# mfkiwl/erlangnetwork-gnsslib-sdr

Hardware: AMD Instinct MI355X
Metric: correlations/sec (1 ms coh) + x real-time, 32-SV L1CA @16.368 Msps (higher is better)
Workload: dtype int8 samples x int8 carrier LUT -> int32 accumulators (exact); NCOs: the reference's fp64 running sums, bit for bit; 1 GPU; BASELINE configs[2]: 32-SV GPS L1CA tracking, 5-tap E/P/L correlators (CORRN=2, CORRD=3), 1 ms coherent, 16.368 Msps int8 IQ, per GPU; channels_per_gpu=32, epochs_per_launch=1000, taps=5, loop=open (frequencies held per launch); see closed_loop (--full), if_broadcast=none (1 GPU)

## Files before the change

erlangnetwork-gnsslib-sdr_amd/csrc/gnsscorr_api.hip:

```cpp
#include <cstdarg>
#include <cstdio>
#include <cstdlib>
#include <cstring>

#include "gnsscorr_ctx.h"

static thread_local char g_err[512] = "";

int gc_fail(int code, const char *fmt, ...)
{
    va_list ap;
    va_start(ap, fmt);
    vsnprintf(g_err, sizeof(g_err), fmt, ap);
    va_end(ap);
    return code;
}

int gc_fail_hip(hipError_t e, const char *what, const char *file, int line)
{
    snprintf(g_err, sizeof(g_err), "HIP error %d (%s) in %s at %s:%d", (int)e, hipGetErrorString(e), what,
             file, line);
    return GNSSCORR_EHIP;
}

extern "C" const char *gnsscorr_last_error(void) { return g_err; }

extern "C" int gnsscorr_device_count(void)
{
    int n = 0;
    if (hipGetDeviceCount(&n) != hipSuccess) return 0;
    return n;
}

static void destroy_handles(gnsscorr_ctx *ctx)
{
    for (auto &kv : ctx->timers)
        for (auto &p : kv.second.pending) { hipEventDestroy(p.first); hipEventDestroy(p.second); }
    for (int i = 0; i < 2; i++)
        for (hipEvent_t e : {ctx->ev_plan[i], ctx->ev_used[i], ctx->ev_corr[i], ctx->ev_fin[i]})
            if (e) hipEventDestroy(e);
    for (hipEvent_t e : {ctx->ev_spec, ctx->ev_chain, ctx->ev_pin[0], ctx->ev_pin[1], ctx->ev_in, ctx->ev_lock})
        if (e) hipEventDestroy(e);
    for (hipEvent_t e : ctx->ev_burst)
        if (e) hipEventDestroy(e);
    for (hipStream_t s : {ctx->stream_plan, ctx->stream_finish, ctx->stream_discover, ctx->stream_in})
        if (s) hipStreamDestroy(s);
    if (ctx->own_stream) hipStreamDestroy(ctx->stream);
}

extern "C" int gnsscorr_create(gnsscorr_ctx **out, int device, void *stream)
{
    if (!out) return gc_fail(GNSSCORR_EINVAL, "gnsscorr_create: null out pointer");
    int ndev = 0;
    GC_HIP(hipGetDeviceCount(&ndev));
    if (device < 0 || device >= ndev)
        return gc_fail(GNSSCORR_EHIP, "gnsscorr_create: device %d not present (%d visible)", device, ndev);
    GC_HIP(hipSetDevice(device));
    gnsscorr_ctx *ctx = new gnsscorr_ctx();
    ctx->device = device;
    hipError_t e = hipSuccess;
    if (stream) {
        ctx->stream = (hipStream_t)stream;
    } else {
        e = hipStreamCreateWithFlags(&ctx->stream, hipStreamNonBlocking);
        ctx->own_stream = e == hipSuccess;
    }
    for (hipStream_t *s : {&ctx->stream_plan, &ctx->stream_finish, &ctx->stream_discover})
        if (e == hipSuccess) e = hipStreamCreateWithFlags(s, hipStreamNonBlocking);
    for (hipEvent_t *ev : {&ctx->ev_spec, &ctx->ev_chain, &ctx->ev_plan[0], &ctx->ev_used[0], &ctx->ev_corr[0], &ctx->ev_fin[0],
                           &ctx->ev_plan[1], &ctx->ev_used[1], &ctx->ev_corr[1], &ctx->ev_fin[1]})
        if (e == hipSuccess) e = hipEventCreateWithFlags(ev, hipEventDisableTiming);
    for (hipEvent_t &ev : ctx->ev_burst)
        if (e == hipSuccess) e = hipEventCreateWithFlags(&ev, hipEventDisableTiming);
    if (e != hipSuccess) {
        destroy_handles(ctx);
        delete ctx;
        return gc_fail_hip(e, "gnsscorr_create: stream / event", __FILE__, __LINE__);
    }
    *out = ctx;
    return GNSSCORR_OK;
}

static void drop_channel_buffers(gnsscorr_ctx *ctx)
{
    gc_acq_free(ctx);
    gc_spec_free(ctx);
    ctx->dchan.reset(); ctx->dcodes.reset(); ctx->dfreqs.reset();
    ctx->state = GcTrkStateBuf();
    ctx->batch = GcBatch();
    ctx->out = GcTrkOut();
    ctx->loop = GcLoop();
    ctx->rx = GcRx();
    ctx->lock_pending = false;
}

extern "C" void gnsscorr_destroy(gnsscorr_ctx *ctx)
{
    if (!ctx) return;
    hipSetDevice(ctx->device);
    gc_quiesce(ctx, true);
    gc_acq_free(ctx);
    gc_spec_free(ctx);
    destroy_handles(ctx);
// ... 497 lines not shown
```

erlangnetwork-gnsslib-sdr_amd/csrc/gnsscorr_compat.hip:

```cpp
#include <cmath>
#include <cstdio>
#include <cstdlib>
#include <cstring>
#include <ctime>
#include <unistd.h>

#include "../../include/sdr_compat.h"
#include "gnsscorr_ctx.h"

#define SDRPRINTF printf

struct GcOnce {
    GcDevBuf<int8_t> data;
    GcDevBuf<int8_t> code;
    GcDevBuf<GcChan> chan;
    GcDevBuf<GcTrkPlan> plan;
    GcDevBuf<GcTrkUnit> unit;
    GcDevBuf<GcUnitSegs> segs;
    GcDevBuf<int> overflow;
    GcDevBuf<double> out;
    GcDevBuf<int> partial;
    GcDevBuf<GcRound> rounds;
    GcDevBuf<unsigned long long> finish;
};
// ... 33 lines not shown
        }
        *remc = gc_code_rem(c, smax, ci);
    }
}

static int corr_unit(gnsscorr_ctx *ctx, const int8_t *ring, uint64_t ringlen, int dtype, double ti,
                     int n, double freq, double phi0, double crate, double coff, const int *s, int ns,
                     const short *codein, int coden, uint64_t buffloc, double *cI, double *cQ)
{
    if (ns < 1 || 1 + 2 * ns > GNSSCORR_MAXTAPS) return gc_fail(GNSSCORR_EINVAL, "correlator: ns %d", ns);
    if (coden < 1 || coden > 1023) return gc_fail(GNSSCORR_EINVAL, "correlator: code length %d", coden);
    if (n < 1) return gc_fail(GNSSCORR_EINVAL, "correlator: n %d", n);
    int rc = once_init(ctx);
    if (rc) return rc;
    GcChan c;
    memset(&c, 0, sizeof(c));
    c.ring = ring; c.ringlen = ringlen; c.code = g_once.code;
    c.dtype = dtype; c.clen = coden; c.nsamp = n; c.ntap = 1 + 2 * ns; c.smax = s[ns - 1];
    c.tapoff[0] = 0;
    for (int k = 0; k < ns; k++) { c.tapoff[1 + 2 * k] = -s[k]; c.tapoff[2 + 2 * k] = s[k]; }
    c.ti = ti;
    GcTrkPlan p;
    memset(&p, 0, sizeof(p));
    p.buffloc = buffloc; p.coff = coff; p.phi0 = phi0; p.carrfreq = freq; p.codefreq = crate; p.n = n;
    static int8_t block[GC_CODEBLOCK];
    gc_build_codeblock(codein, coden, block, &c.nedge, &c.pm1);
    GC_HIP(hipMemcpyAsync(g_once.code, block, GC_CODEBLOCK, hipMemcpyHostToDevice, ctx->stream));
    GC_HIP(hipMemcpyAsync(g_once.chan, &c, sizeof(c), hipMemcpyHostToDevice, ctx->stream));
    GC_HIP(hipMemcpyAsync(g_once.plan, &p, sizeof(p), hipMemcpyHostToDevice, ctx->stream));
    const int nseg = gc_trk_nseg(dtype, n);
    GC_RESERVE(ctx, g_once.partial, (size_t)nseg * 2 * c.ntap);
    GC_RESERVE(ctx, g_once.rounds, (size_t)nseg * GC_MAXR);
    rc = gc_launch_trk_expand(ctx->stream, g_once.chan, g_once.plan, g_once.unit, g_once.segs, nullptr, 1, 1, g_once.rounds,
                              nseg, n, g_once.overflow);
    if (rc) return rc;
    rc = gc_launch_trk_corr(ctx->stream, g_once.chan, g_once.unit, g_once.segs, g_once.rounds, g_once.partial, 1, 1, nseg,
                            c.ntap, dtype, c.ntap, n, c.smax, nullptr);
    if (rc) return rc;
    rc = gc_launch_trk_finish(ctx->stream, g_once.partial, g_once.out, g_once.out + GNSSCORR_MAXTAPS,
                              g_once.out + 2 * GNSSCORR_MAXTAPS, g_once.out + 3 * GNSSCORR_MAXTAPS, g_once.finish, 1, 1, nseg,
                              c.ntap);
    if (rc) return rc;
    double host[2 * GNSSCORR_MAXTAPS];
    int over = 0;
    GC_HIP(hipMemcpyAsync(host, g_once.out, sizeof(host), hipMemcpyDeviceToHost, ctx->stream));
    GC_HIP(hipMemcpyAsync(&over, g_once.overflow, sizeof(int), hipMemcpyDeviceToHost, ctx->stream));
    GC_HIP(hipStreamSynchronize(ctx->stream));
    if (over) {
        GC_HIP(hipMemsetAsync(g_once.overflow, 0, sizeof(int), ctx->stream));
        return gc_fail(GNSSCORR_EINVAL, "correlator: the call spans more code periods (chip step %g x %d samples over %d chips) "
                       "or carrier binades than the NCO tables hold", ti * crate, n, coden);
    }
    memcpy(cI, host, sizeof(double) * c.ntap);
    memcpy(cQ, host + GNSSCORR_MAXTAPS, sizeof(double) * c.ntap);
    return 0;
}

extern "C" {

void correlator(const char *data, int dtype, double ti, int n, double freq, double phi0, double crate,
                double coff, int *s, int ns, double *II, double *QQ, double *remc, double *remp,
                short *codein, int coden)
{
    gnsscorr_ctx *ctx = gnsscorr_default_ctx();
    if (!ctx) { SDRPRINTF("error: correlator: no GPU context (%s)\n", gnsscorr_last_error()); return; }
    std::lock_guard<std::mutex> lk(ctx->mtx);
    if (hipSetDevice(ctx->device) != hipSuccess) { SDRPRINTF("error: correlator: hipSetDevice\n"); return; }
// ... 128 lines not shown
        const int sm = r->sdr->trk.corrp[r->sdr->trk.corrn - 1];
        if (sm > smax_max) smax_max = sm;
    }
    const int nseg = gc_trk_nseg(dtype, max_n);
    int rc = cmb_reserve(ctx, k, nseg);
    if (rc) return rc;
    const double tp0 = g_cprof.on ? CmbProf::now() : 0.0;
    const size_t plan_off = (sizeof(GcChan) * (size_t)k + 63) & ~(size_t)63;
    GcChan *hchan = reinterpret_cast<GcChan *>(q.hstage.p), *dchan = reinterpret_cast<GcChan *>(q.dstage.p);
    GcTrkPlan *hplan = reinterpret_cast<GcTrkPlan *>(q.hstage.p + plan_off), *dplan = reinterpret_cast<GcTrkPlan *>(q.dstage.p + plan_off);
    for (int i = 0; i < k; i++) {
        sdrch_t *sdr = grp[i]->sdr;
        const GcRing &ring = ctx->ring[sdr->ftype == FTYPE2 ? 1 : 0];
        CodeSlot *cs;
        rc = cmb_code(ctx, sdr, grp[i]->codesum, &cs);
        if (rc) return rc;
        GcChan &c = hchan[i];
        memset(&c, 0, sizeof(c));
        c.ring = ring.mem; c.ringlen = ring.ringlen; c.code = cs->dcode;
        c.dtype = dtype; c.clen = sdr->clen; c.nsamp = grp[i]->n; c.ntap = ntap;
        c.smax = sdr->trk.corrp[sdr->trk.corrn - 1];
        c.tapoff[0] = 0;
        for (int t = 0; t < sdr->trk.corrn; t++) { c.tapoff[1 + 2 * t] = -sdr->trk.corrp[t]; c.tapoff[2 + 2 * t] = sdr->trk.corrp[t]; }
        c.ti = sdr->ti;
        c.nedge = cs->nedge; c.pm1 = cs->pm1;
        GcTrkPlan &p = hplan[i];
        memset(&p, 0, sizeof(p));
        p.buffloc = grp[i]->buffloc; p.coff = sdr->trk.oldremcode; p.phi0 = sdr->trk.oldremcarr;
        p.carrfreq = sdr->trk.carrfreq; p.codefreq = sdr->trk.codefreq; p.n = grp[i]->n;
    }
    hipStream_t st = ctx->stream;
    const double tp1 = g_cprof.on ? CmbProf::now() : 0.0;
    GC_HIP(hipMemcpyAsync(q.dstage, q.hstage, plan_off + sizeof(GcTrkPlan) * k, hipMemcpyHostToDevice, st));
    rc = gc_launch_trk_expand(st, dchan, dplan, q.dunit, q.dsegs, nullptr, k, 1, q.drounds, nseg, max_n, q.hover.dev);
    if (rc) return rc;
    rc = gc_launch_trk_corr(st, dchan, q.dunit, q.dsegs, q.drounds, q.dpartial, k, 1, nseg, ntap, dtype, ntap, max_n, smax_max, nullptr);
    if (rc) return rc;
    double *cI = q.hres.dev, *cQ = q.hres.dev + (size_t)q.cap * ntap, *sI = q.dsum, *sQ = q.dsum + (size_t)q.cap * ntap;
    rc = gc_launch_trk_finish(st, q.dpartial, cI, cQ, sI, sQ, q.dfinish, k, 1, nseg, ntap);
    if (rc) return rc;
    const double tp2 = g_cprof.on ? CmbProf::now() : 0.0;
    GC_HIP(hipStreamSynchronize(st));
    const double tp3 = g_cprof.on ? CmbProf::now() : 0.0;
    if (*q.hover) {
        *q.hover = 0;
        return gc_fail(GNSSCORR_EINVAL, "sdrtracking: a period needs more NCO pieces than the tables hold");
    }
    for (int i = 0; i < k; i++) {
        memcpy(grp[i]->cI, q.hres + (size_t)i * ntap, sizeof(double) * ntap);
        memcpy(grp[i]->cQ, q.hres + (size_t)(q.cap + i) * ntap, sizeof(double) * ntap);
    }
    g_cmb_stats[0]++; g_cmb_stats[1] += (unsigned long long)k;
    if ((unsigned long long)k > g_cmb_stats[2]) g_cmb_stats[2] = (unsigned long long)k;
    if (g_cprof.on) {
        const double tp4 = CmbProf::now();
        g_cprof.batches++; g_cprof.reqs += (unsigned long long)k;
        g_cprof.t[0] += tp1 - tp0; g_cprof.t[1] += tp2 - tp1; g_cprof.t[2] += tp3 - tp2; g_cprof.t[3] += tp4 - tp3;
    }
    return 0;
}

void cmb_run(std::vector<TrkReq *> &batch)
{
    const double tr0 = g_cprof.on ? CmbProf::now() : 0.0;
    struct Whole { double t0; ~Whole() { if (g_cprof.on) g_cprof.t[4] += CmbProf::now() - t0; } } whole{tr0};
    gnsscorr_ctx *ctx = gnsscorr_default_ctx();
    auto fail_all = [&](std::vector<TrkReq *> &v, const char *msg) {
// ... 123 lines not shown
```

erlangnetwork-gnsslib-sdr_amd/csrc/gnsscorr_ctx.h:

```cpp
#pragma once

#include <map>
#include <mutex>
#include <string>
#include <utility>
#include <vector>

#include <cstring>
#include "gnsscorr_internal.h"

struct gnsscorr_ctx;
int gc_dev_alloc(gnsscorr_ctx *ctx, void **p, size_t bytes);

template <class T>
struct GcDevBuf {
    T *p = nullptr;
    size_t n = 0;
    GcDevBuf() = default;
    GcDevBuf(GcDevBuf &&o) noexcept : p(o.p), n(o.n) { o.p = nullptr; o.n = 0; }
    GcDevBuf &operator=(GcDevBuf &&o) noexcept
    {
        if (this != &o) { reset(); p = o.p; n = o.n; o.p = nullptr; o.n = 0; }
        return *this;
    }
// ... 65 lines not shown
    double total_ms = 0.0;
    int launches = 0;
};

struct GcAcqWork;
struct GcSpecWork;

struct GcTrkStateBuf {
    GcDevBuf<GcTrkState> buf[2];
    int icur = 0;
    bool touched = true;
    GcTrkState *cur() const { return buf[icur]; }
    GcTrkState *next() const { return buf[icur ^ 1]; }
    void commit() { icur ^= 1; }
};

struct GcTrkOut {
    GcDevBuf<double> dcorrI, dcorrQ;
    GcDevBuf<double> dsumI, dsumQ;
    GcDevBuf<int> nsamp;
    GcDevBuf<int> dnco_overflow;
    GcDevBuf<int> dring_viol;
    size_t units = 0;
    int last_nepoch = 0;
    bool fin_pending = false;
    int fin_slot = 0;
};

struct GcPlanSlot {
    GcDevBuf<GcTrkPlan> plan;
    GcDevBuf<GcTrkUnit> unit;
    GcDevBuf<GcRound> rounds;
    GcDevBuf<GcUnitSegs> segs;
    GcDevBuf<int> partial;
    bool fin_pending = false;
};

struct GcBatch {
    GcPlanSlot slot[2];
    size_t units = 0;
    int nseg = 1;
    GcDevBuf<int> dspec2[2];
    GcDevBuf<unsigned short> detab;
    GcDevBuf<unsigned long long> dfinish;
    bool spec_pending = false;
    bool spec_ahead_valid = false;
    int spec_ahead_buf = 0, spec_ahead_nepoch = 0;
    int spec_last_buf = 0, spec_last_units = 0;
    const void *spec_ahead_state = nullptr;
    int plan_slot = 0;
    bool ahead_valid = false;
    int ahead_nepoch = 0;
};

#define GC_LOOP_AHEAD 3
struct GcLoop {
    GcDevBuf<gnsscorr_loop_t> dloop;
    std::vector<char> isset;
    GcDevBuf<GcStepMeta> dstep_meta;
    GcDevBuf<GcTrkUnit> dstep_unit;
    GcDevBuf<GcUnitSegs> dstep_segs;
    GcDevBuf<GcRound> dstep_rounds;
    GcDevBuf<int> dstep_partial;
    int step_nseg = 0;
    GcPinBuf<unsigned> hostflags;
    int kmax = 1;
    bool sync_hint = false;
    GcDevBuf<gnsscorr_trklog_t> dlog;
    GcDevBuf<int> dlapped;
    GcDevBuf<int> ddone;
    GcDevBuf<uint64_t> dwrpos;
    int run_nper = 0;
    int last_nper = 0;
};

struct GcRx {
// ... 10 lines not shown
    GcPinBuf<unsigned> lock_lost;
};

struct gnsscorr_ctx {
    int device = 0;
    hipStream_t stream = nullptr;
    bool own_stream = false;
    std::mutex mtx;

    GcRing ring[2];

    hipStream_t stream_in = nullptr;
    GcPinBuf<int8_t> pin[2];
    GcDevBuf<uint8_t> dstage[2];
    hipEvent_t ev_pin[2] = {nullptr, nullptr};
    bool pin_busy[2] = {false, false};
    int pin_next = 0;
    hipEvent_t ev_in = nullptr;
    bool in_pending = false;

    int nch = 0;
    std::vector<GcChan> hchan;
    std::vector<gnsscorr_chan_t> hdesc;
    std::vector<std::vector<short>> hcode;
    std::vector<std::vector<double>> hfreq;
    std::vector<std::vector<int>> hcorrp;
    GcDevBuf<GcChan> dchan;
    GcDevBuf<int8_t> dcodes;
    GcDevBuf<double> dfreqs;
    int ntap = 0, smax_max = 0, max_n = 0;
    bool have_dtype[3] = {false, false, false};

    hipStream_t stream_plan = nullptr;
    hipStream_t stream_finish = nullptr;
    hipStream_t stream_discover = nullptr;
    hipEvent_t ev_plan[2] = {};
    hipEvent_t ev_used[2] = {};
    hipEvent_t ev_corr[2] = {};
    hipEvent_t ev_fin[2] = {};
    hipEvent_t ev_spec = nullptr, ev_chain = nullptr;
    GcTrkStateBuf state;
    GcBatch batch;
    GcTrkOut out;
    GcLoop loop;
    hipEvent_t ev_burst[GC_LOOP_AHEAD] = {};
    GcRx rx;
    hipEvent_t ev_lock = nullptr;
    bool lock_pending = false;

    GcAcqWork *acq = nullptr;

    GcSpecWork *spec = nullptr;

    GcDevBuf<signed char> dfec_sym;
    GcDevBuf<unsigned char> dfec_out;
    int fec_parts = 3;

    GcDevBuf<unsigned char> dlock_stage;

    int timing = 0;
    std::map<std::string, GcTimer> timers;

    int poison = -1;
};

struct GcTimed {
    gnsscorr_ctx *ctx;
    hipEvent_t a = nullptr, b = nullptr;
    const char *name;
    hipStream_t st;
// ... 31 lines not shown
```

erlangnetwork-gnsslib-sdr_amd/csrc/gnsscorr_internal.h:

```cpp
#pragma once

#include <hip/hip_runtime.h>
#include <stdint.h>
#include "../../include/gnsscorr.h"
#include "gnsscorr_nco.h"

#define GC_DPI      (2.0*3.1415926535897932)
#define GC_CDIV     32
#define GC_RCPAD    16

typedef const __attribute__((address_space(1))) int8_t *gc_gptr_i8;
typedef unsigned gc_u4v __attribute__((ext_vector_type(4)));
typedef const __attribute__((address_space(1))) gc_u4v *gc_gptr_u4;

struct GcChan {
    const int8_t *ring;
    uint64_t ringlen;
    const int8_t *code;
    int    dtype, clen, nsamp, nsampchip;
    int    ntap, smax;
    int    tapoff[GNSSCORR_MAXTAPS];
    double ti, f_sf, crate, ctime;
    int    nfreq, intg, nfft, grid;
    int    freq_off;
// ... 59 lines not shown
    GcCodeSeg code[GC_NCODE];
};

struct GcAcqRow {
    double rowmax;
    double sum_out;
    double max_out;
    int    argmax;
    int    pad;
};

#define GC_HIP(call)                                                           \
    do {                                                                       \
        hipError_t e_ = (call);                                                \
        if (e_ != hipSuccess) return gc_fail_hip(e_, #call, __FILE__, __LINE__); \
    } while (0)

int gc_fail_hip(hipError_t e, const char *what, const char *file, int line);
int gc_fail(int code, const char *fmt, ...);

#define GC_MAXR 24
struct GcRound {
    int q0, q1;
    short clast, w0;
    int hint;
};

size_t gc_trk_spec_ints(size_t units);
int gc_launch_trk_spec(hipStream_t st, const GcChan *chan, const GcTrkState *state_in, int nch, int nepoch, int *claims,
                       int e_off);
int gc_launch_trk_plan(hipStream_t st, const GcChan *chan, const GcTrkState *state_in, GcTrkState *state_out,
                       GcTrkPlan *plan, int nch, int nepoch, int *claims);
int gc_launch_trk_expand(hipStream_t st, const GcChan *chan, const GcTrkPlan *plan, GcTrkUnit *unit, GcUnitSegs *segs,
                         int *nsamp_out, int nch, int nepoch, GcRound *rounds, int nseg, int max_n, int *nco_overflow);
int gc_launch_trk_corr(hipStream_t st, const GcChan *chan, const GcTrkUnit *unit, const GcUnitSegs *segs,
                       const GcRound *rounds, int *partial, int nch,
                       int nepoch, int nseg, int ntap_stride, int dtype, int ntap, int max_n, int smax_max,
                       const unsigned short *etab);
#define GC_FINISH_SCRATCH (2 * GNSSCORR_MAXTAPS + 1)
int gc_launch_trk_finish(hipStream_t st, const int *partial, double *corrI, double *corrQ, double *sumI,
                         double *sumQ, unsigned long long *scratch, int nch, int nepoch, int nseg, int ntap);
int gc_trk_nseg(int dtype, int max_n);

#define GC_STEP_KMAX 20
struct GcStepMeta {
    int k;
    int kcap;
    int pbase;
    int done;
    int consumed;
    int finished;
    int early;
    int pad;
};
```

erlangnetwork-gnsslib-sdr_amd/csrc/gnsscorr_trk.hip:

```cpp
#include <cstdlib>
#include <type_traits>


#include "gnsscorr_ctx.h"
#include "gnsscorr_ps.h"

namespace {


#define GC_EXP_LANES 64
struct ExpCarTable {
    int *k0;
    GcCarSeg *seg;
    int cap, n, overflow, prevk;
    bool lastzero, bad;
    __device__ void operator()(int k, double x, double d, int )
    {
        const GcCarSeg s = gc_carseg_make(x, d);
        const bool zero = s.fx == 0 && s.dfx == 0;
        if (n > 0 && zero && lastzero) return;
        if (n >= cap) { overflow = 1; return; }
        bad = bad || (n == 0 ? k != 0 : !(prevk < k));
        k0[n] = k;
        seg[n] = s;
// ... 46 lines not shown
        n++;
    }
    __device__ void finish(int nt)
    {
        if (n > 0) {
            flush();
            bad = bad || prev_end != nt;
        }
    }
    __device__ int chip_at(int j, int *w, int *piece) const
    {
        int lo = 0, hi = n - 1;
        while (lo < hi) {
            const int mid = (lo + hi + 1) >> 1;
            if (lds->j0[mid * GC_EXP_LANES + lane] <= j) lo = mid; else hi = mid - 1;
        }
        const int x = lo * GC_EXP_LANES + lane;
        if (w) *w = lds->w[x];
        if (piece) *piece = lo;
        int i = j - lds->j0[x];
        const int cnt = lds->cnt[x];
        if (i < 0) i = 0;
        if (i >= cnt) i = cnt - 1;
        const double d = lds->d[x], y0 = lds->y0[x];
        if (d == 0.0) return (int)y0;
        return (int)fma((double)i, d, y0);
    }
};

__global__ __launch_bounds__(GC_EXP_LANES) void trk_expand_kernel(const GcChan *__restrict__ chan, const GcTrkPlan *__restrict__ plan,
                                  GcTrkUnit *__restrict__ unit, GcUnitSegs *__restrict__ segs,
                                  int *__restrict__ nsamp_out, int nch, int nepoch,
                                  GcRound *__restrict__ rounds, int nseg, int max_n, int nit,
                                  int *__restrict__ nco_overflow)
{
    __shared__ ExpCodeLds slds;
    const int i = blockIdx.x * blockDim.x + threadIdx.x;
    if (i >= nch * nepoch) return;
    const GcChan &c = chan[i / nepoch];
    const GcTrkPlan p = plan[i];
    GcUnitSegs *sg = segs + i;
    GcTrkUnit u;
    const uint64_t a0 = (p.buffloc % c.ringlen) * (uint64_t)c.dtype;
    u.a_al = a0 & ~(uint64_t)15;
    u.head = (int)(a0 - u.a_al);
    u.n = p.n;
    u.G = (u.head + p.n * c.dtype + 15) >> 4;
    u.nt = p.n + 2 * c.smax;
    u.ncar = 0;
    u.ncode = 0;
    u.eq0 = -1;
    u.eq1 = -1;
    if (nsamp_out) nsamp_out[i] = p.n;
    const double ci = __dmul_rn(c.ti, p.codefreq);
    if (!(p.n > 0 && p.n <= max_n && ci > 0.0 && ci < (double)c.clen)) {
        u.n = 0;
        unit[i] = u;
        return;
    }
    ExpCarTable ct{sg->carK0, sg->car, GC_NCAR, 0, 0, 0, false, false};
    ExpCodeTable dt{sg->code, &slds, (int)threadIdx.x, GC_NCODE, 0, 0, 0, false, 0.0, 0.0, 0.0, 0.0, 0, 0, 0};
    {
        GcNcoFast f;
        gc_fast_init(f, gc_carrier_ps(p.carrfreq, c.ti));
        gc_fast_carrier_walk(f, gc_carrier_phis(p.phi0), p.n, ct);
        gc_fast_init(f, ci);
        gc_fast_code_walk(f, gc_code_start(p.coff, c.smax, ci, c.clen), c.clen, u.nt, dt);
        dt.finish(u.nt);
    }
    u.ncar = ct.n;
    u.ncode = dt.n;
    const bool bad = ct.overflow || dt.overflow || ct.n < 1 || dt.n < 1 || ct.bad || dt.bad;
    if (bad) {
// ... 474 lines not shown
    GC_LC(33, 21);
#undef GC_LC
}

void trk_pick_nit()
{
    if (g_trk_nit) return;
    const char *a = getenv("GNSSCORR_TRK_ALGO");
    g_trk_algo = (a && a[0] == 'r') ? 2 : 1;
    const char *e = getenv("GNSSCORR_TRK_NIT");
    g_trk_nit = e ? atoi(e) : 2;
    if (g_trk_algo == 1) {
        if (g_trk_nit != 1 && g_trk_nit != 2) g_trk_nit = 2;
    } else {
        if (g_trk_nit != 2 && g_trk_nit != 4 && g_trk_nit != 8) g_trk_nit = 2;
    }
}

}

int gc_trk_nseg(int dtype, int max_n)
{
    trk_pick_nit();
    const int groups = (15 + max_n * dtype + 15) / 16 + 1;
    const int nit = g_trk_algo == 1 ? trk_ps_nit(dtype, g_trk_nit) : g_trk_nit;
    if (g_trk_algo == 1) {
        const int rounds = (groups + GC_PS_WLANES * nit - 1) / (GC_PS_WLANES * nit);
        return (rounds + GC_MAXR - 1) / GC_MAXR;
    }
    return (groups + 256 * nit - 1) / (256 * nit);
}

int gc_launch_trk_expand(hipStream_t st, const GcChan *chan, const GcTrkPlan *plan, GcTrkUnit *unit, GcUnitSegs *segs,
                         int *nsamp_out, int nch, int nepoch, GcRound *rounds, int nseg, int max_n, int *nco_overflow)
{
    trk_pick_nit();
    const int total = nch * nepoch;
    hipLaunchKernelGGL(trk_expand_kernel, dim3((total + 63) / 64), dim3(64), 0, st, chan, plan, unit, segs, nsamp_out,
                       nch, nepoch, g_trk_algo == 1 ? rounds : (GcRound *)nullptr, nseg, max_n, g_trk_nit, nco_overflow);
    GC_HIP(hipGetLastError());
    return 0;
}

int gc_launch_trk_corr(hipStream_t st, const GcChan *chan, const GcTrkUnit *unit, const GcUnitSegs *segs,
                       const GcRound *rounds, int *partial, int nch,
                       int nepoch, int nseg, int ntap_stride, int dtype, int ntap, int max_n, int smax_max,
                       const unsigned short *etab)
{
    trk_pick_nit();
    if (smax_max > 64) return gc_fail(GNSSCORR_EINVAL, "trk_corr: tap offset %d samples (<= 64 supported)", smax_max);
    static const bool noetab = getenv("GNSSCORR_TRK_NOEDGETAB") != nullptr;
    if (g_trk_algo != 1 || noetab) etab = nullptr;
    if (dtype == 2)
        return launch_corr_taps<2>(st, chan, unit, segs, rounds, partial, nch, nepoch, nseg, ntap_stride, ntap, max_n, smax_max, etab);
    if (dtype == 1)
        return launch_corr_taps<1>(st, chan, unit, segs, rounds, partial, nch, nepoch, nseg, ntap_stride, ntap, max_n, smax_max, etab);
    return gc_fail(GNSSCORR_EINVAL, "trk_corr: dtype %d not 1 or 2", dtype);
}

static int launch_trk_edges(hipStream_t st, const GcChan *chan, const GcTrkUnit *unit, const GcUnitSegs *segs, unsigned short *etab,
                        int nch, int nepoch)
{
    static const bool noetab = getenv("GNSSCORR_TRK_NOEDGETAB") != nullptr;
    trk_pick_nit();
    if (!etab || noetab || g_trk_algo != 1) return 0;
    hipLaunchKernelGGL(trk_edges_kernel, dim3(nch * nepoch), dim3(256), 0, st, chan, unit, segs, etab, nch, nepoch);
    GC_HIP(hipGetLastError());
    return 0;
}

__global__ void trk_ringcheck_kernel(const GcChan *__restrict__ chan, const GcTrkPlan *__restrict__ plan,
                                     const int8_t *ring0, uint64_t wrpos0, uint64_t wrpos1, int nch, int nepoch,
                                     int *__restrict__ viol)
{
    const int i = blockIdx.x * blockDim.x + threadIdx.x;
    if (i >= nch * nepoch) return;
    const int ch = i / nepoch;
    const GcTrkPlan p = plan[i];
    if (p.n <= 0) return;
    const uint64_t wp = chan[ch].ring == ring0 ? wrpos0 : wrpos1, rl = chan[ch].ringlen;
    if (p.buffloc + (uint64_t)p.n > wp || (wp > rl && p.buffloc < wp - rl)) atomicAdd(viol, 1);
}

static int launch_trk_ringcheck(hipStream_t st, const GcChan *chan, const GcTrkPlan *plan, const int8_t *ring0, uint64_t wrpos0,
                            uint64_t wrpos1, int nch, int nepoch, int *viol)
{
    const int total = nch * nepoch;
    hipLaunchKernelGGL(trk_ringcheck_kernel, dim3((total + 255) / 256), dim3(256), 0, st, chan, plan, ring0, wrpos0, wrpos1,
                       nch, nepoch, viol);
    GC_HIP(hipGetLastError());
    return 0;
}

int gc_launch_trk_finish(hipStream_t st, const int *partial, double *corrI, double *corrQ, double *sumI,
                         double *sumQ, unsigned long long *scratch, int nch, int nepoch, int nseg, int ntap)
{
    hipLaunchKernelGGL(trk_finish_kernel, dim3(nch, (nepoch + 255) / 256), dim3(256), 0, st, partial, corrI, corrQ,
                       sumI, sumQ, scratch, nepoch, nseg, ntap);
    GC_HIP(hipGetLastError());
    return 0;
}

int gc_drain(gnsscorr_ctx *ctx)
{
    for (hipStream_t s : {ctx->stream_plan, ctx->stream_finish, ctx->stream_discover, ctx->stream})
        GC_HIP(hipStreamSynchronize(s));
    ctx->out.fin_pending = false;
    for (GcPlanSlot &s : ctx->batch.slot) s.fin_pending = false;
    return GNSSCORR_OK;
}

int gc_quiesce(gnsscorr_ctx *ctx, bool ingest)
{
    if (ingest && ctx->stream_in) GC_HIP(hipStreamSynchronize(ctx->stream_in));
    GC_TRY(gc_drain(ctx));
    ctx->batch.ahead_valid = false;
    ctx->state.touched = true;
    return GNSSCORR_OK;
}

int gc_loop_take_state(gnsscorr_ctx *ctx)
{
    if (ctx->batch.ahead_valid || ctx->out.fin_pending) return gc_quiesce(ctx);
    ctx->state.touched = true;
    return GNSSCORR_OK;
}

int gc_outputs_ready(gnsscorr_ctx *ctx)
{
    if (ctx->out.fin_pending) GC_HIP(hipStreamWaitEvent(ctx->stream, ctx->ev_fin[ctx->out.fin_slot], 0));
    return GNSSCORR_OK;
}

int gc_ensure_trk_outputs(gnsscorr_ctx *ctx, int nperiod)
{
    GcTrkOut &o = ctx->out;
    const size_t units = (size_t)ctx->nch * nperiod;
    if (units <= o.units) return GNSSCORR_OK;
// ... 3 lines not shown
    GC_RESERVE(ctx, o.dcorrQ, units * ctx->ntap);
    GC_RESERVE(ctx, o.nsamp, units);
    GC_RESERVE(ctx, o.dsumI, (size_t)ctx->nch * ctx->ntap);
    GC_RESERVE(ctx, o.dsumQ, (size_t)ctx->nch * ctx->ntap);
    for (GcDevBuf<int> *c : {&o.dnco_overflow, &o.dring_viol}) {
        if (*c) continue;
        GC_RESERVE(ctx, *c, 1);
        GC_HIP(hipMemsetAsync(*c, 0, sizeof(int), ctx->stream));
    }
    o.units = units;
    return GNSSCORR_OK;
}

static int ensure_batch_buffers(gnsscorr_ctx *ctx, int nepoch)
{
    GcBatch &b = ctx->batch;
    const size_t units = (size_t)ctx->nch * nepoch;
    if (units <= b.units) return GNSSCORR_OK;
    GC_TRY(gc_drain(ctx));
    b.ahead_valid = false;
    b.spec_ahead_valid = false;
    b.units = 0;
    b.nseg = 1;
    for (int i = 0; i < ctx->nch; i++) {
        const int s = gc_trk_nseg(ctx->hchan[i].dtype, ctx->max_n);
        if (s > b.nseg) b.nseg = s;
    }
    for (GcPlanSlot &s : b.slot) {
        GC_RESERVE(ctx, s.plan, units);
        GC_RESERVE(ctx, s.partial, units * b.nseg * 2 * ctx->ntap);
        GC_RESERVE(ctx, s.unit, units);
        GC_RESERVE(ctx, s.rounds, units * b.nseg * GC_MAXR);
        GC_RESERVE(ctx, s.segs, units);
    }
    for (int i = 0; i < 2; i++) GC_RESERVE(ctx, b.dspec2[i], gc_trk_spec_ints(units));
    GC_RESERVE(ctx, b.detab, units * GC_EDGTAB);
    GC_RESERVE(ctx, b.dfinish, (size_t)ctx->nch * GC_FINISH_SCRATCH);
    GC_HIP(hipMemsetAsync(b.dfinish, 0, sizeof(unsigned long long) * ctx->nch * GC_FINISH_SCRATCH, ctx->stream));
    b.units = units;
    return GNSSCORR_OK;
}

static int plan_into(gnsscorr_ctx *ctx, int s, int nepoch)
{
    GcBatch &b = ctx->batch;
    GcPlanSlot &sl = b.slot[s];
    hipStream_t ps = ctx->stream_plan;
    if (sl.fin_pending) GC_HIP(hipStreamWaitEvent(ps, ctx->ev_fin[s], 0));
    const GcTrkState *sin = ctx->state.cur();
    int buf;
    if (b.spec_pending) GC_HIP(hipStreamWaitEvent(ps, ctx->ev_spec, 0));
    if (b.spec_ahead_valid && !ctx->state.touched && b.spec_ahead_nepoch == nepoch && b.spec_ahead_state == (const void *)sin) {
        buf = b.spec_ahead_buf;
    } else {
        buf = 0;
        GcTimed t(ctx, "trk_spec", ps);
        GC_TRY(gc_launch_trk_spec(ps, ctx->dchan, sin, ctx->nch, nepoch, b.dspec2[buf], 0));
    }
    b.spec_ahead_valid = false;
    b.spec_pending = false;
    b.spec_last_buf = buf;
    b.spec_last_units = ctx->nch * nepoch;
    GC_HIP(hipEventRecord(ctx->ev_chain, ps));
    GC_HIP(hipStreamWaitEvent(ctx->stream_discover, ctx->ev_chain, 0));
    {
        GcTimed t(ctx, "trk_spec", ctx->stream_discover);
        GC_TRY(gc_launch_trk_spec(ctx->stream_discover, ctx->dchan, sin, ctx->nch, nepoch, b.dspec2[buf ^ 1], nepoch));
        GC_HIP(hipEventRecord(ctx->ev_spec, ctx->stream_discover));
    }
    b.spec_pending = true;
    b.spec_ahead_valid = true;
    b.spec_ahead_buf = buf ^ 1;
    b.spec_ahead_nepoch = nepoch;
    b.spec_ahead_state = (const void *)ctx->state.next();
    {
        GcTimed t(ctx, "trk_plan", ps);
        GC_TRY(gc_launch_trk_plan(ps, ctx->dchan, sin, ctx->state.next(), sl.plan, ctx->nch, nepoch, b.dspec2[buf]));
    }
    GC_HIP(hipEventRecord(ctx->ev_plan[s], ps));
    return GNSSCORR_OK;
}

static int correlate_slot(gnsscorr_ctx *ctx, int s, int nepoch, const uint64_t wr[2])
{
    GcBatch &b = ctx->batch;
    GcPlanSlot &sl = b.slot[s];
    {
        GcTimed t(ctx, "trk_expand");
        GC_TRY(gc_launch_trk_expand(ctx->stream, ctx->dchan, sl.plan, sl.unit, sl.segs, ctx->out.nsamp, ctx->nch, nepoch,
                                    sl.rounds, b.nseg, ctx->max_n, ctx->out.dnco_overflow));
    }
    GC_TRY(launch_trk_ringcheck(ctx->stream, ctx->dchan, sl.plan, (const int8_t *)ctx->ring[0].mem, wr[0], wr[1], ctx->nch,
                                nepoch, ctx->out.dring_viol));
    {
        GcTimed t(ctx, "trk_edges");
        GC_TRY(launch_trk_edges(ctx->stream, ctx->dchan, sl.unit, sl.segs, b.detab, ctx->nch, nepoch));
    }
    for (int dtype = 1; dtype <= 2; dtype++) {
        if (!ctx->have_dtype[dtype]) continue;
        GcTimed t(ctx, "trk_corr");
        GC_TRY(gc_launch_trk_corr(ctx->stream, ctx->dchan, sl.unit, sl.segs, sl.rounds, sl.partial, ctx->nch, nepoch, b.nseg,
                                  ctx->ntap, dtype, ctx->ntap, ctx->max_n, ctx->smax_max, b.detab));
    }
    GC_HIP(hipEventRecord(ctx->ev_corr[s], ctx->stream));
    return GNSSCORR_OK;
}

static int finish_slot(gnsscorr_ctx *ctx, int s, int nepoch)
{
    GcBatch &b = ctx->batch;
    GcTrkOut &o = ctx->out;
    hipStream_t fs = ctx->stream_finish;
    GC_HIP(hipStreamWaitEvent(fs, ctx->ev_corr[s], 0));
    GcTimed t(ctx, "trk_finish", fs);
    GC_TRY(gc_launch_trk_finish(fs, b.slot[s].partial, o.dcorrI, o.dcorrQ, o.dsumI, o.dsumQ, b.dfinish, ctx->nch, nepoch,
                                b.nseg, ctx->ntap));
    GC_HIP(hipEventRecord(ctx->ev_fin[s], fs));
    b.slot[s].fin_pending = true;
    o.fin_pending = true;
    o.fin_slot = s;
    return GNSSCORR_OK;
}

extern "C" int gnsscorr_trk_run(gnsscorr_ctx *ctx, int nepoch)
{
    if (!ctx || nepoch <= 0) return gc_fail(GNSSCORR_EINVAL, "trk_run: nepoch %d", nepoch);
    if (!ctx->nch) return gc_fail(GNSSCORR_ESTATE, "trk_run: no channels set");
    GC_HIP(hipSetDevice(ctx->device));
    GC_TRY(gc_ensure_trk_outputs(ctx, nepoch));
    GC_TRY(ensure_batch_buffers(ctx, nepoch));
    uint64_t wr[2];
    GC_TRY(gc_ring_positions(ctx, wr));
    GcBatch &b = ctx->batch;
    hipStream_t ps = ctx->stream_plan;
    const int cur = b.plan_slot;
    if (!(b.ahead_valid && b.ahead_nepoch == nepoch)) {
        if (b.ahead_valid) {
            GC_HIP(hipStreamSynchronize(ps));
            b.ahead_valid = false;
        }
        GC_HIP(hipEventRecord(ctx->ev_used[cur], ctx->stream));
        GC_HIP(hipStreamWaitEvent(ps, ctx->ev_used[cur], 0));
        GC_TRY(plan_into(ctx, cur, nepoch));
    }
    GC_HIP(hipStreamWaitEvent(ctx->stream, ctx->ev_plan[cur], 0));
    GC_TRY(correlate_slot(ctx, cur, nepoch, wr));
    b.ahead_valid = false;
    ctx->state.commit();
    b.plan_slot ^= 1;
    if (!ctx->state.touched) {
        GC_HIP(hipStreamWaitEvent(ps, ctx->ev_corr[b.plan_slot], 0));
        GC_TRY(plan_into(ctx, b.plan_slot, nepoch));
        b.ahead_valid = true;
        b.ahead_nepoch = nepoch;
    }
    ctx->state.touched = false;
    GC_TRY(finish_slot(ctx, cur, nepoch));
    ctx->out.last_nepoch = nepoch;
    ctx->loop.last_nper = 0;
    return GNSSCORR_OK;
}

int gc_nco_check(gnsscorr_ctx *ctx)
{
    GcTrkOut &o = ctx->out;
    int n = 0, v = 0;
    GC_HIP(hipMemcpy(&v, o.dring_viol, sizeof(int), hipMemcpyDeviceToHost));
    if (v) {
        GC_HIP(hipMemset(o.dring_viol, 0, sizeof(int)));
        return gc_fail(GNSSCORR_ESTATE, "tracking: %d (channel, period) units lay outside what the IF ring holds "
                       "(beyond the write position, or overwritten since): their sums are not the stream's", v);
    }
    GC_HIP(hipMemcpy(&n, o.dnco_overflow, sizeof(int), hipMemcpyDeviceToHost));
    if (!n) return GNSSCORR_OK;
    GC_HIP(hipMemset(o.dnco_overflow, 0, sizeof(int)));
    return gc_fail(GNSSCORR_EINVAL, "tracking: %d (channel, period) units need more NCO pieces than the tables hold "
                   "(more than two code periods per call, or a carrier crossing more than %d binades); their sums are zero",
                   n, GC_NCAR);
}

extern "C" int gnsscorr_trk_fetch(gnsscorr_ctx *ctx, double *trkII, double *trkQQ, int *nsamp_out)
{
    if (!ctx || !ctx->out.last_nepoch) return gc_fail(GNSSCORR_ESTATE, "trk_fetch: no completed trk_run");
    GC_HIP(hipSetDevice(ctx->device));
// ... 68 lines not shown
```

Baseline: 307.8 million correlations/s.

## Move expand/edges to a prepare stream and fold ring check into expand

Splits the per-launch work so trk_expand and trk_edges run on a new prepare stream, with the edge table made per-slot, letting the next slot's preparation overlap the current correlation on the main stream. The separate ring-check kernel is removed and its bounds check moves into the expand kernel, dropping one launch. The spec kernel now shares the finish stream, and the cross-stream dependencies are rewired through new ev_prep events. This adds event-wait complexity and a risk of ordering mistakes; the per-slot edge tables also need more memory.

```diff
diff --git a/erlangnetwork-gnsslib-sdr_amd/csrc/gnsscorr_api.hip b/erlangnetwork-gnsslib-sdr_amd/csrc/gnsscorr_api.hip
--- a/erlangnetwork-gnsslib-sdr_amd/csrc/gnsscorr_api.hip
+++ b/erlangnetwork-gnsslib-sdr_amd/csrc/gnsscorr_api.hip
@@ -37,13 +37,13 @@
     for (auto &kv : ctx->timers)
         for (auto &p : kv.second.pending) { hipEventDestroy(p.first); hipEventDestroy(p.second); }
     for (int i = 0; i < 2; i++)
-        for (hipEvent_t e : {ctx->ev_plan[i], ctx->ev_used[i], ctx->ev_corr[i], ctx->ev_fin[i]})
+        for (hipEvent_t e : {ctx->ev_plan[i], ctx->ev_used[i], ctx->ev_prep[i], ctx->ev_corr[i], ctx->ev_fin[i]})
             if (e) hipEventDestroy(e);
     for (hipEvent_t e : {ctx->ev_spec, ctx->ev_chain, ctx->ev_pin[0], ctx->ev_pin[1], ctx->ev_in, ctx->ev_lock})
         if (e) hipEventDestroy(e);
     for (hipEvent_t e : ctx->ev_burst)
         if (e) hipEventDestroy(e);
-    for (hipStream_t s : {ctx->stream_plan, ctx->stream_finish, ctx->stream_discover, ctx->stream_in})
+    for (hipStream_t s : {ctx->stream_plan, ctx->stream_finish, ctx->stream_prepare, ctx->stream_in})
         if (s) hipStreamDestroy(s);
     if (ctx->own_stream) hipStreamDestroy(ctx->stream);
 }
@@ -65,10 +65,10 @@
         e = hipStreamCreateWithFlags(&ctx->stream, hipStreamNonBlocking);
         ctx->own_stream = e == hipSuccess;
     }
-    for (hipStream_t *s : {&ctx->stream_plan, &ctx->stream_finish, &ctx->stream_discover})
+    for (hipStream_t *s : {&ctx->stream_plan, &ctx->stream_finish, &ctx->stream_prepare})
         if (e == hipSuccess) e = hipStreamCreateWithFlags(s, hipStreamNonBlocking);
-    for (hipEvent_t *ev : {&ctx->ev_spec, &ctx->ev_chain, &ctx->ev_plan[0], &ctx->ev_used[0], &ctx->ev_corr[0], &ctx->ev_fin[0],
-                           &ctx->ev_plan[1], &ctx->ev_used[1], &ctx->ev_corr[1], &ctx->ev_fin[1]})
+    for (hipEvent_t *ev : {&ctx->ev_spec, &ctx->ev_chain, &ctx->ev_plan[0], &ctx->ev_used[0], &ctx->ev_prep[0], &ctx->ev_corr[0],
+                           &ctx->ev_fin[0], &ctx->ev_plan[1], &ctx->ev_used[1], &ctx->ev_prep[1], &ctx->ev_corr[1], &ctx->ev_fin[1]})
         if (e == hipSuccess) e = hipEventCreateWithFlags(ev, hipEventDisableTiming);
     for (hipEvent_t &ev : ctx->ev_burst)
         if (e == hipSuccess) e = hipEventCreateWithFlags(&ev, hipEventDisableTiming);
diff --git a/erlangnetwork-gnsslib-sdr_amd/csrc/gnsscorr_compat.hip b/erlangnetwork-gnsslib-sdr_amd/csrc/gnsscorr_compat.hip
--- a/erlangnetwork-gnsslib-sdr_amd/csrc/gnsscorr_compat.hip
+++ b/erlangnetwork-gnsslib-sdr_amd/csrc/gnsscorr_compat.hip
@@ -89,7 +89,7 @@
     GC_RESERVE(ctx, g_once.partial, (size_t)nseg * 2 * c.ntap);
     GC_RESERVE(ctx, g_once.rounds, (size_t)nseg * GC_MAXR);
     rc = gc_launch_trk_expand(ctx->stream, g_once.chan, g_once.plan, g_once.unit, g_once.segs, nullptr, 1, 1, g_once.rounds,
-                              nseg, n, g_once.overflow);
+                              nseg, n, g_once.overflow, nullptr, 0, 0, nullptr);
     if (rc) return rc;
     rc = gc_launch_trk_corr(ctx->stream, g_once.chan, g_once.unit, g_once.segs, g_once.rounds, g_once.partial, 1, 1, nseg,
                             c.ntap, dtype, c.ntap, n, c.smax, nullptr);
@@ -284,7 +284,8 @@
     hipStream_t st = ctx->stream;
     const double tp1 = g_cprof.on ? CmbProf::now() : 0.0;
     GC_HIP(hipMemcpyAsync(q.dstage, q.hstage, plan_off + sizeof(GcTrkPlan) * k, hipMemcpyHostToDevice, st));
-    rc = gc_launch_trk_expand(st, dchan, dplan, q.dunit, q.dsegs, nullptr, k, 1, q.drounds, nseg, max_n, q.hover.dev);
+    rc = gc_launch_trk_expand(st, dchan, dplan, q.dunit, q.dsegs, nullptr, k, 1, q.drounds, nseg, max_n, q.hover.dev, nullptr, 0, 0,
+                              nullptr);
     if (rc) return rc;
     rc = gc_launch_trk_corr(st, dchan, q.dunit, q.dsegs, q.drounds, q.dpartial, k, 1, nseg, ntap, dtype, ntap, max_n, smax_max, nullptr);
     if (rc) return rc;
diff --git a/erlangnetwork-gnsslib-sdr_amd/csrc/gnsscorr_ctx.h b/erlangnetwork-gnsslib-sdr_amd/csrc/gnsscorr_ctx.h
--- a/erlangnetwork-gnsslib-sdr_amd/csrc/gnsscorr_ctx.h
+++ b/erlangnetwork-gnsslib-sdr_amd/csrc/gnsscorr_ctx.h
@@ -121,6 +121,7 @@
     GcDevBuf<GcTrkUnit> unit;
     GcDevBuf<GcRound> rounds;
     GcDevBuf<GcUnitSegs> segs;
+    GcDevBuf<unsigned short> etab;
     GcDevBuf<int> partial;
     bool fin_pending = false;
 };
@@ -130,7 +131,6 @@
     size_t units = 0;
     int nseg = 1;
     GcDevBuf<int> dspec2[2];
-    GcDevBuf<unsigned short> detab;
     GcDevBuf<unsigned long long> dfinish;
     bool spec_pending = false;
     bool spec_ahead_valid = false;
@@ -207,10 +207,11 @@
     bool have_dtype[3] = {false, false, false};
 
     hipStream_t stream_plan = nullptr;
+    hipStream_t stream_prepare = nullptr;
     hipStream_t stream_finish = nullptr;
-    hipStream_t stream_discover = nullptr;
     hipEvent_t ev_plan[2] = {};
     hipEvent_t ev_used[2] = {};
+    hipEvent_t ev_prep[2] = {};
     hipEvent_t ev_corr[2] = {};
     hipEvent_t ev_fin[2] = {};
     hipEvent_t ev_spec = nullptr, ev_chain = nullptr;
diff --git a/erlangnetwork-gnsslib-sdr_amd/csrc/gnsscorr_internal.h b/erlangnetwork-gnsslib-sdr_amd/csrc/gnsscorr_internal.h
--- a/erlangnetwork-gnsslib-sdr_amd/csrc/gnsscorr_internal.h
+++ b/erlangnetwork-gnsslib-sdr_amd/csrc/gnsscorr_internal.h
@@ -115,7 +115,8 @@
 int gc_launch_trk_plan(hipStream_t st, const GcChan *chan, const GcTrkState *state_in, GcTrkState *state_out,
                        GcTrkPlan *plan, int nch, int nepoch, int *claims);
 int gc_launch_trk_expand(hipStream_t st, const GcChan *chan, const GcTrkPlan *plan, GcTrkUnit *unit, GcUnitSegs *segs,
-                         int *nsamp_out, int nch, int nepoch, GcRound *rounds, int nseg, int max_n, int *nco_overflow);
+                         int *nsamp_out, int nch, int nepoch, GcRound *rounds, int nseg, int max_n, int *nco_overflow,
+                         const int8_t *ring0, uint64_t wrpos0, uint64_t wrpos1, int *ring_viol);
 int gc_launch_trk_corr(hipStream_t st, const GcChan *chan, const GcTrkUnit *unit, const GcUnitSegs *segs,
                        const GcRound *rounds, int *partial, int nch,
                        int nepoch, int nseg, int ntap_stride, int dtype, int ntap, int max_n, int smax_max,
diff --git a/erlangnetwork-gnsslib-sdr_amd/csrc/gnsscorr_trk.hip b/erlangnetwork-gnsslib-sdr_amd/csrc/gnsscorr_trk.hip
--- a/erlangnetwork-gnsslib-sdr_amd/csrc/gnsscorr_trk.hip
+++ b/erlangnetwork-gnsslib-sdr_amd/csrc/gnsscorr_trk.hip
@@ -102,13 +102,18 @@
                                   GcTrkUnit *__restrict__ unit, GcUnitSegs *__restrict__ segs,
                                   int *__restrict__ nsamp_out, int nch, int nepoch,
                                   GcRound *__restrict__ rounds, int nseg, int max_n, int nit,
-                                  int *__restrict__ nco_overflow)
+                                  int *__restrict__ nco_overflow, const int8_t *ring0, uint64_t wrpos0, uint64_t wrpos1,
+                                  int *__restrict__ ring_viol)
 {
     __shared__ ExpCodeLds slds;
     const int i = blockIdx.x * blockDim.x + threadIdx.x;
     if (i >= nch * nepoch) return;
     const GcChan &c = chan[i / nepoch];
     const GcTrkPlan p = plan[i];
+    if (ring_viol && p.n > 0) {
+        const uint64_t wp = c.ring == ring0 ? wrpos0 : wrpos1, rl = c.ringlen;
+        if (p.buffloc + (uint64_t)p.n > wp || (wp > rl && p.buffloc < wp - rl)) atomicAdd(ring_viol, 1);
+    }
     GcUnitSegs *sg = segs + i;
     GcTrkUnit u;
     const uint64_t a0 = (p.buffloc % c.ringlen) * (uint64_t)c.dtype;
@@ -649,12 +654,14 @@
 }
 
 int gc_launch_trk_expand(hipStream_t st, const GcChan *chan, const GcTrkPlan *plan, GcTrkUnit *unit, GcUnitSegs *segs,
-                         int *nsamp_out, int nch, int nepoch, GcRound *rounds, int nseg, int max_n, int *nco_overflow)
+                         int *nsamp_out, int nch, int nepoch, GcRound *rounds, int nseg, int max_n, int *nco_overflow,
+                         const int8_t *ring0, uint64_t wrpos0, uint64_t wrpos1, int *ring_viol)
 {
     trk_pick_nit();
     const int total = nch * nepoch;
     hipLaunchKernelGGL(trk_expand_kernel, dim3((total + 63) / 64), dim3(64), 0, st, chan, plan, unit, segs, nsamp_out,
-                       nch, nepoch, g_trk_algo == 1 ? rounds : (GcRound *)nullptr, nseg, max_n, g_trk_nit, nco_overflow);
+                       nch, nepoch, g_trk_algo == 1 ? rounds : (GcRound *)nullptr, nseg, max_n, g_trk_nit, nco_overflow,
+                       ring0, wrpos0, wrpos1, ring_viol);
     GC_HIP(hipGetLastError());
     return 0;
 }
@@ -686,29 +693,6 @@
     return 0;
 }
 
-__global__ void trk_ringcheck_kernel(const GcChan *__restrict__ chan, const GcTrkPlan *__restrict__ plan,
-                                     const int8_t *ring0, uint64_t wrpos0, uint64_t wrpos1, int nch, int nepoch,
-                                     int *__restrict__ viol)
-{
-    const int i = blockIdx.x * blockDim.x + threadIdx.x;
-    if (i >= nch * nepoch) return;
-    const int ch = i / nepoch;
-    const GcTrkPlan p = plan[i];
-    if (p.n <= 0) return;
-    const uint64_t wp = chan[ch].ring == ring0 ? wrpos0 : wrpos1, rl = chan[ch].ringlen;
-    if (p.buffloc + (uint64_t)p.n > wp || (wp > rl && p.buffloc < wp - rl)) atomicAdd(viol, 1);
-}
-
-static int launch_trk_ringcheck(hipStream_t st, const GcChan *chan, const GcTrkPlan *plan, const int8_t *ring0, uint64_t wrpos0,
-                            uint64_t wrpos1, int nch, int nepoch, int *viol)
-{
-    const int total = nch * nepoch;
-    hipLaunchKernelGGL(trk_ringcheck_kernel, dim3((total + 255) / 256), dim3(256), 0, st, chan, plan, ring0, wrpos0, wrpos1,
-                       nch, nepoch, viol);
-    GC_HIP(hipGetLastError());
-    return 0;
-}
-
 int gc_launch_trk_finish(hipStream_t st, const int *partial, double *corrI, double *corrQ, double *sumI,
                          double *sumQ, unsigned long long *scratch, int nch, int nepoch, int nseg, int ntap)
 {
@@ -720,7 +704,7 @@
 
 int gc_drain(gnsscorr_ctx *ctx)
 {
-    for (hipStream_t s : {ctx->stream_plan, ctx->stream_finish, ctx->stream_discover, ctx->stream})
+    for (hipStream_t s : {ctx->stream_plan, ctx->stream_prepare, ctx->stream_finish, ctx->stream})
         GC_HIP(hipStreamSynchronize(s));
     ctx->out.fin_pending = false;
     for (GcPlanSlot &s : ctx->batch.slot) s.fin_pending = false;
@@ -790,9 +774,9 @@
         GC_RESERVE(ctx, s.unit, units);
         GC_RESERVE(ctx, s.rounds, units * b.nseg * GC_MAXR);
         GC_RESERVE(ctx, s.segs, units);
+        GC_RESERVE(ctx, s.etab, units * GC_EDGTAB);
     }
     for (int i = 0; i < 2; i++) GC_RESERVE(ctx, b.dspec2[i], gc_trk_spec_ints(units));
-    GC_RESERVE(ctx, b.detab, units * GC_EDGTAB);
     GC_RESERVE(ctx, b.dfinish, (size_t)ctx->nch * GC_FINISH_SCRATCH);
     GC_HIP(hipMemsetAsync(b.dfinish, 0, sizeof(unsigned long long) * ctx->nch * GC_FINISH_SCRATCH, ctx->stream));
     b.units = units;
@@ -804,7 +788,7 @@
     GcBatch &b = ctx->batch;
     GcPlanSlot &sl = b.slot[s];
     hipStream_t ps = ctx->stream_plan;
-    if (sl.fin_pending) GC_HIP(hipStreamWaitEvent(ps, ctx->ev_fin[s], 0));
+    GC_HIP(hipStreamWaitEvent(ps, ctx->ev_prep[s], 0));
     const GcTrkState *sin = ctx->state.cur();
     int buf;
     if (b.spec_pending) GC_HIP(hipStreamWaitEvent(ps, ctx->ev_spec, 0));
@@ -820,11 +804,12 @@
     b.spec_last_buf = buf;
     b.spec_last_units = ctx->nch * nepoch;
     GC_HIP(hipEventRecord(ctx->ev_chain, ps));
-    GC_HIP(hipStreamWaitEvent(ctx->stream_discover, ctx->ev_chain, 0));
+    hipStream_t ds = ctx->stream_finish;
+    GC_HIP(hipStreamWaitEvent(ds, ctx->ev_chain, 0));
     {
-        GcTimed t(ctx, "trk_spec", ctx->stream_discover);
-        GC_TRY(gc_launch_trk_spec(ctx->stream_discover, ctx->dchan, sin, ctx->nch, nepoch, b.dspec2[buf ^ 1], nepoch));
-        GC_HIP(hipEventRecord(ctx->ev_spec, ctx->stream_discover));
+        GcTimed t(ctx, "trk_spec", ds);
+        GC_TRY(gc_launch_trk_spec(ds, ctx->dchan, sin, ctx->nch, nepoch, b.dspec2[buf ^ 1], nepoch));
+        GC_HIP(hipEventRecord(ctx->ev_spec, ds));
     }
     b.spec_pending = true;
     b.spec_ahead_valid = true;
@@ -839,26 +824,38 @@
     return GNSSCORR_OK;
 }
 
-static int correlate_slot(gnsscorr_ctx *ctx, int s, int nepoch, const uint64_t wr[2])
+static int prepare_slot(gnsscorr_ctx *ctx, int s, int nepoch, const uint64_t wr[2])
 {
     GcBatch &b = ctx->batch;
     GcPlanSlot &sl = b.slot[s];
+    hipStream_t hs = ctx->stream_prepare;
+    GC_HIP(hipStreamWaitEvent(hs, ctx->ev_plan[s], 0));
+    GC_HIP(hipStreamWaitEvent(hs, ctx->ev_corr[s], 0));
     {
-        GcTimed t(ctx, "trk_expand");
-        GC_TRY(gc_launch_trk_expand(ctx->stream, ctx->dchan, sl.plan, sl.unit, sl.segs, ctx->out.nsamp, ctx->nch, nepoch,
-                                    sl.rounds, b.nseg, ctx->max_n, ctx->out.dnco_overflow));
-    }
-    GC_TRY(launch_trk_ringcheck(ctx->stream, ctx->dchan, sl.plan, (const int8_t *)ctx->ring[0].mem, wr[0], wr[1], ctx->nch,
-                                nepoch, ctx->out.dring_viol));
+        GcTimed t(ctx, "trk_expand", hs);
+        GC_TRY(gc_launch_trk_expand(hs, ctx->dchan, sl.plan, sl.unit, sl.segs, ctx->out.nsamp, ctx->nch, nepoch, sl.rounds,
+                                    b.nseg, ctx->max_n, ctx->out.dnco_overflow, (const int8_t *)ctx->ring[0].mem, wr[0], wr[1],
+                                    ctx->out.dring_viol));
+    }
     {
-        GcTimed t(ctx, "trk_edges");
-        GC_TRY(launch_trk_edges(ctx->stream, ctx->dchan, sl.unit, sl.segs, b.detab, ctx->nch, nepoch));
-    }
+        GcTimed t(ctx, "trk_edges", hs);
+        GC_TRY(launch_trk_edges(hs, ctx->dchan, sl.unit, sl.segs, sl.etab, ctx->nch, nepoch));
+    }
+    GC_HIP(hipEventRecord(ctx->ev_prep[s], hs));
+    return GNSSCORR_OK;
+}
+
+static int correlate_slot(gnsscorr_ctx *ctx, int s, int nepoch)
+{
+    GcBatch &b = ctx->batch;
+    GcPlanSlot &sl = b.slot[s];
+    GC_HIP(hipStreamWaitEvent(ctx->stream, ctx->ev_prep[s], 0));
+    if (sl.fin_pending) GC_HIP(hipStreamWaitEvent(ctx->stream, ctx->ev_fin[s], 0));
     for (int dtype = 1; dtype <= 2; dtype++) {
         if (!ctx->have_dtype[dtype]) continue;
         GcTimed t(ctx, "trk_corr");
         GC_TRY(gc_launch_trk_corr(ctx->stream, ctx->dchan, sl.unit, sl.segs, sl.rounds, sl.partial, ctx->nch, nepoch, b.nseg,
-                                  ctx->ntap, dtype, ctx->ntap, ctx->max_n, ctx->smax_max, b.detab));
+                                  ctx->ntap, dtype, ctx->ntap, ctx->max_n, ctx->smax_max, sl.etab));
     }
     GC_HIP(hipEventRecord(ctx->ev_corr[s], ctx->stream));
     return GNSSCORR_OK;
@@ -901,13 +898,12 @@
         GC_HIP(hipStreamWaitEvent(ps, ctx->ev_used[cur], 0));
         GC_TRY(plan_into(ctx, cur, nepoch));
     }
-    GC_HIP(hipStreamWaitEvent(ctx->stream, ctx->ev_plan[cur], 0));
-    GC_TRY(correlate_slot(ctx, cur, nepoch, wr));
+    GC_TRY(prepare_slot(ctx, cur, nepoch, wr));
+    GC_TRY(correlate_slot(ctx, cur, nepoch));
     b.ahead_valid = false;
     ctx->state.commit();
     b.plan_slot ^= 1;
     if (!ctx->state.touched) {
-        GC_HIP(hipStreamWaitEvent(ps, ctx->ev_corr[b.plan_slot], 0));
         GC_TRY(plan_into(ctx, b.plan_slot, nepoch));
         b.ahead_valid = true;
         b.ahead_nepoch = nepoch;
```

Result: no change. 309.8 million correlations/s, median of 6 (+0.6%).
